# viniciusvidal2/slam-sensor-fusion

Hardware: AMD Instinct MI355X
Metric: scans_per_s_200k_scan_vs_10M_map (higher is better)
Workload: dtype f32 points / f64 accumulation

## Files before the change

### include/slamfusion.h

```cpp
#ifndef SLAMFUSION_H
#define SLAMFUSION_H
#include <stdint.h>

#ifdef __cplusplus
extern "C" {
#endif

#define SF_VERSION 210

typedef enum {
    SF_OK = 0,
    SF_ERR_INVALID = -1,
    SF_ERR_HIP = -2,
    SF_ERR_NOMEM = -3,
    SF_ERR_STATE = -4,
    SF_ERR_OVERFLOW = -5,
    SF_ERR_COMM = -6
} sf_status;

typedef struct sf_ctx sf_ctx;
typedef struct sf_cloud sf_cloud;
typedef struct sf_map sf_map;
typedef struct sf_icp sf_icp;

// ... 150 lines not shown
int sf_icp_align_batch_async(sf_icp *icp, int mode);
int sf_icp_fetch_results(sf_icp *icp, sf_icp_result *out);
int sf_icp_fetch_previous(sf_icp *icp, sf_icp_result *out);
int sf_icp_use_graph(sf_icp *icp, int on);
int sf_icp_graph_counts(sf_icp *icp, int64_t *captures, int64_t *launches);
int sf_icp_set_fused(sf_icp *icp, int on);
int sf_icp_fused_count(sf_icp *icp, int64_t *launches);
int sf_icp_fused_redone(sf_icp *icp, int64_t *redone);
int sf_icp_test_inject_barrier_timeout(sf_icp *icp);
#define SF_ORDER_AUTO 0
#define SF_ORDER_AS_GIVEN 1
#define SF_ORDER_CELL 2
int sf_icp_set_query_order(sf_icp *icp, int order);
int sf_icp_set_nn_reuse(sf_icp *icp, int on);
int sf_icp_set_wide_scan_points(sf_icp *icp, int64_t points);
int sf_icp_set_pipeline(sf_icp *icp, int on);
int sf_icp_set_tile_search(sf_icp *icp, int mode);
int sf_icp_tile_info(sf_icp *icp, int64_t out[12]);
int sf_icp_set_freeze(sf_icp *icp, int on);
int sf_icp_set_freeze_params(sf_icp *icp, float guard_scale, float guard_min, float guard_max, int max_tries, int from_launch);
int sf_icp_freeze_stats(sf_icp *icp, int64_t out[5]);
int sf_icp_set_defer_search(sf_icp *icp, int on);
int sf_icp_defer_stats(sf_icp *icp, int64_t out[2]);
int sf_icp_set_neighbour_research(sf_icp *icp, int from_launch);
int sf_icp_neighbour_stats(sf_icp *icp, int64_t out[3]);
int sf_icp_neighbour_gap_stats(sf_icp *icp, int64_t out[4]);
#define SF_ROBUST_NONE 0
#define SF_ROBUST_HUBER 1
#define SF_ROBUST_CAUCHY 2
#define SF_ROBUST_TUKEY 3
#define SF_ROBUST_GM 4
int sf_icp_set_robust_kernel(sf_icp *icp, int kind, double k);

#define SF_COV_EIG_EPS 1e-12
#define SF_COV_FEW_CORR 1
#define SF_COV_SINGULAR 2
#define SF_COV_DEGENERATE_TRANS 4
#define SF_COV_DEGENERATE_ROT 8
typedef struct {
    double info[36];
    double cov[36];
    double sigma2, sigma2_hat, weight_sum;
    double trans_info[3], trans_dir[9];
    double rot_info[3], rot_dir[9];
    int64_t n_corr;
    int32_t flags;
// ... 202 lines not shown
```

### slam_sensor_fusion_amd/api.py

```python
import atexit
import ctypes as C
import os
import weakref

import numpy as np

_HERE = os.path.dirname(os.path.abspath(__file__))
LIB_PATH = os.path.join(_HERE, "lib", "libslamfusion.so")

SF_ICP_REF_CPP, SF_ICP_O3D_P2P, SF_ICP_P2PLANE = 0, 1, 2
SF_VOXEL_PCL, SF_VOXEL_O3D, SF_VOXEL_PCL64 = 0, 1, 2
SF_FLAG_VOXEL_OVERFLOW = 1
SF_ICP_FLAG_FEW_CORR, SF_ICP_FLAG_SINGULAR, SF_ICP_FLAG_SHARD_STALE, SF_ICP_FLAG_BARRIER_TIMEOUT = 1, 2, 4, 8
PROF_NN, PROF_REDUCE, PROF_COLLECTIVE, PROF_SOLVE, PROF_SHARD_BUILD = 0, 1, 2, 3, 4
SF_ERR_COMM = -6
MODES = {"ref_cpp": SF_ICP_REF_CPP, "o3d_p2p": SF_ICP_O3D_P2P, "p2plane": SF_ICP_P2PLANE}
ROBUST_KINDS = {"none": 0, "huber": 1, "cauchy": 2, "tukey": 3, "gm": 4}


class SlamFusionError(RuntimeError):
    pass


class IcpResult(C.Structure):
# ... 782 lines not shown
        return {"froze": a[0], "thawed": a[1], "failed": a[2], "active_queries": a[3], "frozen_at_end": a[4]}

    def set_defer_search(self, on=True):
        _check(self.lib.sf_icp_set_defer_search(self.h, C.c_int(int(bool(on)))))

    def set_neighbour_research(self, from_launch=2):
        _check(self.lib.sf_icp_set_neighbour_research(self.h, C.c_int(int(from_launch))))

    def neighbour_stats(self):
        a = (C.c_int64 * 3)()
        _check(self.lib.sf_icp_neighbour_stats(self.h, a))
        return {"served": a[0], "not_served": a[1], "waves_searched": a[2]}

    def neighbour_gap_stats(self):
        a = (C.c_int64 * 4)()
        _check(self.lib.sf_icp_neighbour_gap_stats(self.h, a))
        return {"served": a[0], "not_served": a[1], "waves_searched": a[2], "by_gap": a[3]}

    def defer_stats(self):
        a = (C.c_int64 * 2)()
        _check(self.lib.sf_icp_defer_stats(self.h, a))
        return {"deferred_queries": a[0], "capped_waves": a[1]}

    def set_query_order(self, order="auto"):
        _check(self.lib.sf_icp_set_query_order(self.h, C.c_int({"auto": 0, "as_given": 1, "cell": 2}[order])))

    def align(self, mode="ref_cpp"):
        r = IcpResult()
        _check(self.lib.sf_icp_align(self.h, C.c_int(MODES[mode]), C.byref(r)))
        return r.as_dict()

    def align_batch(self, mode="p2plane"):
        arr = (IcpResult * self.batch)()
        _check(self.lib.sf_icp_align_batch(self.h, C.c_int(MODES[mode]), arr))
        self._prev_batch, self._last_batch = getattr(self, "_last_batch", None), self.batch
        return [r.as_dict() for r in arr]

    def align_batch_async(self, mode="p2plane"):
        _check(self.lib.sf_icp_align_batch_async(self.h, C.c_int(MODES[mode])))
        self._prev_batch, self._last_batch = getattr(self, "_last_batch", None), self.batch

    def fetch_results(self, raw=False):
        arr = (IcpResult * int(getattr(self, "_last_batch", None) or self.batch))()
        _check(self.lib.sf_icp_fetch_results(self.h, arr))
        return arr if raw else [r.as_dict() for r in arr]

# ... 639 lines not shown
```

### slam_sensor_fusion_amd/csrc/sf_icp.hip

```cpp
#include "sf_common.hpp"
#include "sf_nn.hpp"
#include "sf_tile.hpp"
#include "sf_order.hpp"
#include "sf_p2p.hpp"

#include <cfloat>
#include <cstdlib>
#include <cmath>
#include <vector>
#include <mutex>
#include <string>

namespace {

constexpr int BLK = 256;
constexpr int NREC_P2P = 17;
constexpr int NREC_PLANE = 30;
constexpr int REC_STRIDE = 32;

struct IcpState {
    double T[16];
    double rec[REC_STRIDE];
    double fitness, rmse, prev_fitness, prev_rmse;
    float last_error, err_pending;
// ... 1653 lines not shown
    const int r = (int)blockIdx.x, b = (int)blockIdx.y;
    if (A.st[b].done) return;
    const int fmode = A.fz[b].mode;
    if (fmode == 2) {
        const int64_t total = A.fz[b].n_active;
        for (int bx = r; (int64_t)bx * FZ_CAP < total; bx += FZ_FEW) {
            nn_red_fz_row<Q, SHARD>(g, w, A, b, bx, 2);
            __syncthreads();
        }
        return;
    }
    for (int bx = r; bx < A.nblocks; bx += FZ_FEW) {
        nn_red_fz_row<Q, SHARD>(g, w, A, b, bx, fmode);
        __syncthreads();
    }
}


#ifndef SF_DF_WCAP
#define SF_DF_WCAP 8
#endif
constexpr int DF_WCAP = SF_DF_WCAP;
constexpr int DF_CAPPED = 255;
static_assert((BLK / 64) * DF_WCAP <= FZ_CAP && DF_WCAP < DF_CAPPED, "a row defers fewer queries than it could list as active");
struct DeferBufs {
    uint8_t *cnt;
    uint16_t *ids;
    double *part;
    uint32_t *stat;
};

template <int Q>
__global__ __launch_bounds__(BLK, NN_RED_WAVES) void k_nn_red_df(SfGrid g, SfWindow w, const float *__restrict__ X0x, const float *__restrict__ X0y, const float *__restrict__ X0z,
                                                                 int n, const IcpState *__restrict__ st, float thr, double *__restrict__ partials, int nblocks,
                                                                 float4 *__restrict__ qcache, int64_t cache_n, uint32_t *__restrict__ stats, DeferBufs df)
{
    constexpr int MODE = 2;
    constexpr int NREC = NREC_PLANE;
    const int L = blockIdx.y * gridDim.x + blockIdx.x;
    const int kk = L >> 3;
    const int b = kk % (int)gridDim.y;
    const int bx = (L & 7) * ((int)gridDim.x >> 3) + kk / (int)gridDim.y;
    if (bx >= nblocks) return;
    const IcpState *S = st + b;
    if (S->done) return;
    __shared__ sf::WaveNN nn_ws[BLK / 64];
    __shared__ double stage[BLK / 64][32];
    const int wv = threadIdx.x >> 6, lane = threadIdx.x & 63;
    const size_t seg = ((size_t)b * nblocks + bx) * (BLK / 64) + wv;
    LanePair P[Q];
    bool need[Q];
#pragma unroll
    for (int u = 0; u < Q; ++u) need[u] = false;
    const bool attempted = qcache != nullptr && S->cache_live != 0 && S->n_research >= VERIFY_FROM_SEARCH;
    bool fast = false;
    uint32_t listed = 0;
    if (attempted) {
        const float m_now = (float)S->motion;
#pragma unroll
        for (int u = 0; u < Q; ++u) {
            const int slot = bx * (BLK * Q) + u * BLK + (int)threadIdx.x;
            const QueryIn q = query_in<MODE, false>(X0x, X0y, X0z, n, b, S, 0.0f, 0.0f, nullptr, qcache, cache_n, true, slot, n);
            sf::NNHit hit, seed;
            float4 tn;
            need[u] = reuse_certificate(q.valid, q.qx, q.qy, q.qz, thr, m_now, q.e, q.c1, q.c2, hit, tn, seed);
            if (g.nbr != nullptr && S->n_research >= g.nbr_from) {
                const bool tried = need[u] && seed.j >= 0;
                int served = 0;
                if (tried) {
                    served = table_serve<MODE>(g, q, thr, m_now, seed, qcache, cache_n, hit, tn);
                    need[u] = served == 0;
                }
                if (stats) table_count(stats, tried, served);
            }
            P[u] = make_pair(q, hit, tn);
        }
        uint32_t failing = 0;
// ... 98 lines not shown
                const LanePair A1 = nn_pair<MODE, false, false>(g, w, X0x, X0y, X0z, n, b, S, thr, 0.0f, 0.0f, nullptr, qcache, cache_n, slot, n, &nn_ws[wv], stats, nullptr, false);
#pragma unroll
                for (int h = 0; h < 2; ++h) {
                    double v[16];
#pragma unroll
                    for (int k = 0; k < 16; ++k) v[k] = 0.0;
                    const PairTerms t = pair_terms<MODE>(A1);
                    add_half<MODE>(t, h, v);
                    const double t0 = wave_reduce_16(v);
                    if ((lane & 3) == 0) fstage[wv][16 * h + (lane >> 2)] = t0;
                }
            } else if (lane < 32) {
                fstage[wv][lane] = 0.0;
            }
            __syncthreads();
            if (threadIdx.x < 32) acc += ((fstage[0][threadIdx.x] + fstage[1][threadIdx.x]) + fstage[2][threadIdx.x]) + fstage[3][threadIdx.x];
            __syncthreads();
        }
    }
    if (threadIdx.x < REC_STRIDE) df.part[((size_t)b * FZ_FEW + r) * REC_STRIDE + threadIdx.x] = threadIdx.x < NREC_PLANE ? acc : 0.0;
    __syncthreads();
    if (threadIdx.x == 0) {
        if (n_listed) atomicAdd(&df.stat[0], n_listed);
        if (capped) atomicAdd(&df.stat[1], capped);
    }
}

__device__ __forceinline__ void add_deferred_rows(const double *__restrict__ df_part, int b, double *rec)
{
    if (threadIdx.x < NREC_PLANE) {
        double v = 0.0;
#pragma unroll
        for (int r = 0; r < FZ_FEW; ++r) v += df_part[((size_t)b * FZ_FEW + r) * REC_STRIDE + threadIdx.x];
        rec[threadIdx.x] += v;
    }
    __syncthreads();
}

template <int STRIDE, int NCOL, int NT>
__device__ __forceinline__ void reduce_columns(const double *__restrict__ part, int nrows, double *out)
{
    constexpr int NS = 8;
    static_assert(NT % 128 == 0 && NT / 128 >= 1 && NT / 128 <= NS && NCOL <= 128, "slices of 128 columns");
    __shared__ double sl[NS][128];
    const int c = threadIdx.x & 127;
    for (int sidx = threadIdx.x >> 7; sidx < NS; sidx += NT / 128) {
        double v0 = 0, v1 = 0, v2 = 0, v3 = 0;
// ... 212 lines not shown
    const int b = blockIdx.x;
    IcpState *S = st + b;
    if (S->done) return;
    FreezeState *F = fb.fz + b;
    __shared__ double rec[REC_STRIDE];
    freeze_fold<RBLK>(S, F, b, partials, nblocks, nblocks, fb, rec);
    if (fb.df_part) add_deferred_rows(fb.df_part, b, rec);
    if (threadIdx.x == 0) {
        for (int c = 0; c < NREC_PLANE; ++c) S->rec[c] = rec[c];
        double To[12];
#pragma unroll
        for (int i = 0; i < 12; ++i) To[i] = S->T[i];
        const double m0 = S->motion;
        double upd[12];
        solve_plane(S, rec, n_src, K, upd);
        track_motion(S, To, boxp[b]);
        freeze_after_update(S, F, m0, S->motion, fp, request, upd);
    }
}

__global__ void k_fz_init(FreezeState *__restrict__ fz, int batch, uint32_t *__restrict__ df_stat)
{
    const int b = blockIdx.x * blockDim.x + threadIdx.x;
    if (b == 0) df_stat[0] = df_stat[1] = 0u;
    if (b >= batch) return;
    FreezeState *F = fz + b;
    F->mode = 0; F->tries = 0; F->froze = 0; F->thawed = 0; F->n_active = 0; F->guard = 0.0f; F->launch_mode = 0; F->motion0 = 0.0;
}

constexpr int SBLK = 256;
template <int MODE>
__global__ __launch_bounds__(SBLK) void k_reduce_only(IcpState *__restrict__ st, const double *__restrict__ partials, int nblocks, double *__restrict__ xchg,
                                                      const uint32_t *__restrict__ own_off, int qpl, FreezeBufs fb)
{
    constexpr int NREC = MODE == 2 ? NREC_PLANE : NREC_P2P;
    const int b = blockIdx.x;
    __shared__ double rec[REC_STRIDE];
    if (st[b].done) {
        if (threadIdx.x < REC_STRIDE) xchg[(size_t)b * REC_STRIDE + threadIdx.x] = 0.0;
        return;
    }
    const int rows = own_off ? (int)((own_off[b + 1] - own_off[b] + BLK * qpl - 1) / (BLK * qpl)) : nblocks;
    if (MODE == 2 && fb.fz) freeze_fold<SBLK>(st + b, fb.fz + b, b, partials, nblocks, rows, fb, rec);
    else reduce_partials<NREC, SBLK>(partials + (size_t)b * nblocks * REC_STRIDE, rows, rec);
    if (MODE == 2 && fb.df_part) add_deferred_rows(fb.df_part, b, rec);
    if (threadIdx.x < REC_STRIDE) xchg[(size_t)b * REC_STRIDE + threadIdx.x] = rec[threadIdx.x];
}
// ... 534 lines not shown
    int own_nblocks = 1;
    sf::DevBuf d_box;
    int last_mode = 0;
    bool fused = true;
    bool last_fused = false;
    sf::DevBuf bar;
    int fused_limit[4] = {-1, -1, -1, -1};
    double fused_share = 0.0;
    int64_t fused_redone = 0;
    bool inject_timeout = false;
    int64_t fused_launches = 0;
    IcpState *h_pin = nullptr;
    size_t h_pin_cap = 0;
    bool use_graph = false;
    int64_t graph_captures = 0, graph_replays = 0;
    struct GraphKey {
        int mode = -1, iters = -1, batch = -1, window = -1, ordered = -1, reuse = -1, robust_kind = -1, cov_on = -1;
        int64_t n = -1;
        const void *map = nullptr;
        uint64_t map_generation = 0, epochs = 0;
        uint64_t nbr_stamp = 0;
        const void *nbr = nullptr;
        int nbr_from = 0;
        float max_corr = 0, accept = 0, eps = 0;
        double robust_k = 0;
        double cov_prm[5] = {0, 0, 0, 0, 0};
        bool operator==(const GraphKey &o) const
        {
            return mode == o.mode && iters == o.iters && batch == o.batch && window == o.window && ordered == o.ordered && reuse == o.reuse && n == o.n && map == o.map &&
                   map_generation == o.map_generation && epochs == o.epochs && nbr_stamp == o.nbr_stamp && nbr == o.nbr && nbr_from == o.nbr_from && max_corr == o.max_corr && accept == o.accept && eps == o.eps &&
                   robust_kind == o.robust_kind && robust_k == o.robust_k && cov_on == o.cov_on && std::memcmp(cov_prm, o.cov_prm, sizeof(cov_prm)) == 0;
        }
    };
    struct LaneMeta {
        bool valid = false;
        bool cov = false;
        int batch = 0, mode = 0;
        std::vector<double> inits;
        int src_set = 0;
        uint64_t src_version = 0;
    };
    struct Lane {
        sf::DevBuf X;
        sf::DevBuf qcache;
        sf::DevBuf Xq, qkeys, qkeys2, qidx, qidx2;
        sf::DevBuf corr;
        sf::DevBuf state, d_inits, partials;
        sf::DevBuf fz_state, fz_part, fz_cnt, fz_ids, fz_all;
        sf::DevBuf df_cnt, df_ids, df_part, df_stat;
        sf::DevBuf qtkey, tseg, tile_stats;
        sf::DevBuf cov_part, cov_out;
        hipGraphExec_t graph_exec = nullptr;
        GraphKey graph_key;
// ... 48 lines not shown
    const void *mark_map = nullptr;
    SfWindow mark_window{};
    bool profiling = false;
    std::vector<hipEvent_t> ev;
    size_t ev_used = 0;
    int64_t prof_launches = 0;
    double prof_ms = 0;
    std::vector<float> prof_each;
    std::vector<int> ev_kind;
    std::vector<float> prof_phase[SF_PROF_KINDS];
    sf::DevBuf nn_stats;
    int freeze = 1;
    FreezeParams fz_prm{8.0f, 2.0e-5f, 3.0e-4f, 3};
    int fz_from = 5;
    bool fz_from_auto = true;
    int fz_fetches = 0;
    int fz_step = 0;
    int nbr_from = SF_NBR_FROM;
    bool nbr_active = false;
    int64_t nbr_stats_first = 0;
    uint64_t mark_nbr_stamp = 0;
    int defer = 1;
    bool df_planned = false;
    int64_t nn_stats_used = 0;
    static constexpr int64_t NN_STATS_CAP = 1024;
    int robust_kind = SF_ROBUST_NONE;
    double robust_k = 0.0;
    int cov_on = 0;
    CovArg cov_arg{0.0, 0.0, 0.0, 0.0, 0.0};
    bool prev_cov_ok = false;
    int tile_mode = 0;
    bool tile_on = false;
    sf::SfTiles tiles{};
};

namespace {

using Lane = sf_icp::Lane;
using SrcSet = sf_icp::SrcSet;
float *soa(sf::DevBuf &b, int64_t total, int axis) { return b.as<float>() + (size_t)axis * (size_t)total; }
const float *queries(sf_icp *icp, int axis)
{
    Lane &ln = icp->cur(); SrcSet &ss = icp->src();
    if (icp->shard) return soa(ln.Xq, icp->own_total, axis);
    return soa(icp->ordered ? ln.Xq : ss.X0, ss.plane, axis);
}
// ... 334 lines not shown
        (void)e;
    }
    ~ProfScope()
    {
        if (!icp->profiling) return;
        hipError_t e = hipEventRecord(icp->ev[icp->ev_used + 1], icp->ctx->stream);
        (void)e;
        icp->ev_used += 2;
    }
};

void prof_collect(sf_icp *icp)
{
    for (size_t k = 0; k + 1 < icp->ev_used; k += 2) {
        float ms = 0;
        if (hipEventElapsedTime(&ms, icp->ev[k], icp->ev[k + 1]) != hipSuccess) continue;
        const int kind = k / 2 < icp->ev_kind.size() ? icp->ev_kind[k / 2] : SF_PROF_NN;
        if (kind == SF_PROF_NN) { icp->prof_ms += ms; icp->prof_launches += 1; icp->prof_each.push_back(ms); }
        else if (kind > 0 && kind < SF_PROF_KINDS) icp->prof_phase[kind].push_back(ms);
    }
    icp->ev_used = 0;
}

sf_icp::GraphKey graph_key_now(const sf_icp *icp, int mode)
{
    const Lane &ln = icp->cur(); const SrcSet &ss = icp->src();
    sf_icp::GraphKey k;
    k.mode = mode; k.iters = icp->prm.num_iters; k.batch = ss.batch; k.window = icp->map->window.kind; k.ordered = (int)icp->ordered | ((int)icp->tile_on << 1); k.reuse = (int)icp->reuse | (icp->freeze << 1) | (icp->fz_from << 3) | (icp->defer << 16);
    k.n = (mode == SF_ICP_REF_CPP && ss.batch == 1) ? -ss.n_cap : ss.n;
    k.map = (const void *)icp->map;
    k.map_generation = icp->map->generation;
    if (icp->nbr_active) { k.nbr_stamp = icp->map->nbr_stamp; k.nbr = icp->map->nbr.p; k.nbr_from = icp->nbr_from; }
    k.robust_kind = robust_on(icp, mode) ? icp->robust_kind : SF_ROBUST_NONE; k.robust_k = robust_on(icp, mode) ? icp->robust_k : 0.0;
    k.cov_on = icp->cov_on;
    if (icp->cov_on) { const double cp[5] = {icp->cov_arg.sensor_sigma, icp->cov_arg.thr_t, icp->cov_arg.thr_r, icp->cov_arg.infl_t, icp->cov_arg.infl_r}; std::memcpy(k.cov_prm, cp, sizeof(cp)); }
    k.max_corr = icp->prm.max_corr; k.accept = icp->prm.accept; k.eps = icp->prm.eps + icp->fz_prm.guard_scale * 1.0e-3f + icp->fz_prm.guard_min + icp->fz_prm.guard_max + (float)icp->fz_prm.max_tries;
    const sf::DevBuf *bufs[] = {&ss.X0, &ss.X0r, &ln.X, &ln.Xq, &ln.qcache, &ln.corr, &ln.state, &ln.partials, &icp->d_box, &ss.d_boxes, &ss.n_dev,
                                &icp->map->pts4, &icp->map->nrm4, &icp->map->cell_start, &icp->map->d_window, &ln.fz_state, &ln.fz_part, &ln.fz_cnt, &ln.fz_ids, &ln.fz_all, &ln.df_cnt, &ln.df_ids, &ln.df_part, &ln.df_stat, &ln.tseg, &ln.tile_stats, &ln.cov_part, &ln.cov_out};
    k.epochs = (uint64_t)ss.plane;
    for (const sf::DevBuf *b : bufs) k.epochs = (k.epochs * 1000003ull + b->epoch) * 1000003ull + (uint64_t)(uintptr_t)b->p;
    return k;
}

SfGrid grid_for(const sf_icp *icp)
{
    SfGrid g = icp->map->grid;
    g.nbr = icp->nbr_active ? icp->map->nbr.as<uint4>() : nullptr;
    g.nbr_from = icp->nbr_from;
    return g;
}

int nbr_prepare(sf_icp *icp, int mode)
{
    sf_map *m = icp->map;
    const SrcSet &ss = icp->src();
// ... 83 lines not shown
}

bool freeze_on(const sf_icp *icp, int mode)
{
    const SrcSet &ss = icp->src();
    const int64_t nq = icp->shard ? icp->own_total : ss.n * ss.batch;
    const bool wanted = icp->freeze == 2 || (icp->freeze == 1 && nq >= FREEZE_AUTO_MIN_QUERIES);
    return mode == SF_ICP_P2PLANE && wanted && !robust_on(icp, mode) && icp->reuse && ss.qpl == SF_WIDE_QPL && icp->map->window.kind == 0 && icp->prm.num_iters > icp->fz_from + 1 &&
           icp->fz_from >= VERIFY_FROM_SEARCH;
}

int freeze_alloc(sf_icp *icp)
{
    Lane &ln = icp->cur(); SrcSet &ss = icp->src();
    const size_t rows = (size_t)ss.batch * (size_t)std::max(ss.nblocks_nn, icp->shard ? icp->own_nblocks : 0);
    SF_TRY(ln.fz_state.reserve(sizeof(FreezeState) * (size_t)ss.batch));
    SF_TRY(ln.fz_part.reserve(sizeof(double) * FZ_NMOM * rows));
    SF_TRY(ln.fz_cnt.reserve(sizeof(uint32_t) * rows));
    SF_TRY(ln.fz_ids.reserve(sizeof(uint16_t) * FZ_CAP * rows));
    SF_TRY(ln.fz_all.reserve(sizeof(uint32_t) * FZ_CAP * rows));
    SF_TRY(ln.df_cnt.reserve(sizeof(uint8_t) * (BLK / 64) * rows));
    SF_TRY(ln.df_ids.reserve(sizeof(uint16_t) * (BLK / 64) * DF_WCAP * rows));
    SF_TRY(ln.df_part.reserve(sizeof(double) * REC_STRIDE * FZ_FEW * (size_t)ss.batch));
    SF_TRY(ln.df_stat.reserve(sizeof(uint32_t) * 2));
    return SF_OK;
}

FreezeBufs freeze_bufs(sf_icp *icp, bool on, bool deferred = false)
{
    Lane &ln = icp->cur();
    FreezeBufs fb;
    fb.fz = on ? ln.fz_state.as<FreezeState>() : nullptr;
    fb.mom_part = ln.fz_part.as<double>();
    fb.act_cnt = ln.fz_cnt.as<uint32_t>();
    fb.act_ids = ln.fz_ids.as<uint16_t>();
    fb.act_all = ln.fz_all.as<uint32_t>();
    fb.df_part = deferred ? ln.df_part.as<double>() : nullptr;
    return fb;
}

DeferBufs defer_bufs(sf_icp *icp)
{
    Lane &ln = icp->cur();
    DeferBufs d;
    d.cnt = ln.df_cnt.as<uint8_t>();
    d.ids = ln.df_ids.as<uint16_t>();
    d.part = ln.df_part.as<double>();
    d.stat = ln.df_stat.as<uint32_t>();
    return d;
}

bool defer_now(const sf_icp *icp, int mode, int k)
{
    return freeze_on(icp, mode) && icp->defer != 0 && !icp->shard && k >= VERIFY_FROM_SEARCH && k + 1 == icp->fz_from;
}

bool defer_planned(const sf_icp *icp, int mode) { return defer_now(icp, mode, icp->fz_from - 1); }

void launch_nn_deferred(sf_icp *icp, uint32_t *stats)
{
    Lane &ln = icp->cur(); SrcSet &ss = icp->src();
    sf_map *m = icp->map;
    hipLaunchKernelGGL((k_nn_deferred<SF_WIDE_QPL>), dim3((unsigned)FZ_FEW, (unsigned)ss.batch), dim3(BLK), 0, icp->ctx->stream, grid_for(icp), m->window, queries(icp, 0), queries(icp, 1), queries(icp, 2),
                       (int)ss.n, ln.state.as<IcpState>(), o3d_thr(icp), ss.nblocks_nn, ln.qcache.as<float4>(), icp->cache_n, stats, defer_bufs(icp));
}

void launch_nn_red_df(sf_icp *icp)
{
    Lane &ln = icp->cur(); SrcSet &ss = icp->src();
    sf_map *m = icp->map;
    const int nb = ss.nblocks_nn;
    const dim3 grid((unsigned)((nb + 7) & ~7), (unsigned)ss.batch), blk(BLK);
    ProfScope ps(icp);
    uint32_t *stats = nullptr;
    if (icp->profiling && icp->nn_stats.p && icp->nn_stats_used < sf_icp::NN_STATS_CAP) stats = icp->nn_stats.as<uint32_t>() + NN_STATS_PER * NN_STATS_SHARDS * icp->nn_stats_used++;
    hipLaunchKernelGGL((k_nn_red_df<SF_WIDE_QPL>), grid, blk, 0, icp->ctx->stream, grid_for(icp), m->window, queries(icp, 0), queries(icp, 1), queries(icp, 2), (int)ss.n, ln.state.as<IcpState>(),
                       o3d_thr(icp), ln.partials.as<double>(), nb, ln.qcache.as<float4>(), icp->cache_n, stats, defer_bufs(icp));
    launch_nn_deferred(icp, stats);
}

void launch_nn_red_fz(sf_icp *icp, bool sharded, bool few)
{
    Lane &ln = icp->cur(); SrcSet &ss = icp->src();
    sf_map *m = icp->map;
    const int nb = sharded ? icp->own_nblocks : ss.nblocks_nn;
    const dim3 grid_full((unsigned)((nb + 7) & ~7), (unsigned)ss.batch), grid_few((unsigned)FZ_FEW, (unsigned)ss.batch), blk(BLK);
    ProfScope ps(icp);
    FzArgs A;
    A.X0x = queries(icp, 0); A.X0y = queries(icp, 1); A.X0z = queries(icp, 2);
    A.n = (int)ss.n;
    A.st = ln.state.as<IcpState>();
    A.thr = o3d_thr(icp); A.xlo = icp->xlo; A.xhi = icp->xhi;
    A.partials = ln.partials.as<double>();
    A.nblocks = nb;
    A.own_off = icp->own_off.as<uint32_t>();
    A.qcache = ln.qcache.as<float4>();
    A.cache_n = icp->cache_n;
    A.stats = nullptr;
    if (icp->profiling && icp->nn_stats.p && icp->nn_stats_used < sf_icp::NN_STATS_CAP) A.stats = icp->nn_stats.as<uint32_t>() + NN_STATS_PER * NN_STATS_SHARDS * icp->nn_stats_used++;
    A.fz = ln.fz_state.as<FreezeState>();
// ... 96 lines not shown
int enqueue_align(sf_icp *icp, int mode)
{
    Lane &ln = icp->cur(); SrcSet &ss = icp->src();
    sf_map *m = icp->map;
    hipStream_t s = icp->ctx->stream;
    IcpState *st = ln.state.as<IcpState>();
    double *part = ln.partials.as<double>();
    const int K = icp->prm.num_iters;
    const int B = ss.batch;
    const int n = (int)ss.n;
    if (mode == SF_ICP_O3D_P2P) {
        for (int k = 0; k <= K; ++k) {
            if (tile_launch(icp, k)) launch_tile_search<1>(icp, false);
            else launch_nn_red<1>(icp);
            hipLaunchKernelGGL(k_reduce_solve<1>, dim3(B), dim3(RBLK), 0, s, st, part, ss.nblocks_nn, n, k, K, ss.d_boxes.as<ScanBox>());
        }
    } else if (mode == SF_ICP_P2PLANE) {
        const bool fz = freeze_on(icp, mode);
        if (fz) {
            hipLaunchKernelGGL(k_fz_init, dim3(nblk(B, 64)), dim3(64), 0, s, ln.fz_state.as<FreezeState>(), B, ln.df_stat.as<uint32_t>());
        }
        const bool wide = ss.qpl > 1 && !icp->shard;
        for (int k = 0; k < K; ++k) {
            const bool q1 = wide && k < VERIFY_FROM_SEARCH;
            const bool df = !q1 && defer_now(icp, mode, k);
            if (fz && k >= icp->fz_from) launch_nn_red_fz(icp, false, k > icp->fz_from);
            else if (tile_launch(icp, k)) launch_tile_search<2>(icp, q1);
            else if (df) launch_nn_red_df(icp);
            else launch_nn_red<2>(icp, false, q1);
            if (fz && k + 1 >= icp->fz_from)
                hipLaunchKernelGGL(k_reduce_solve_fz, dim3(B), dim3(RBLK), 0, s, st, part, q1 ? ss.nblocks : ss.nblocks_nn, n, K, ss.d_boxes.as<ScanBox>(), freeze_bufs(icp, true, df),
                                   icp->fz_prm, (int)(k + 2 < K));
            else if (q1)
                hipLaunchKernelGGL(k_reduce_solve<2>, dim3(B), dim3(RBLK), 0, s, st, part, ss.nblocks, n, k, K, ss.d_boxes.as<ScanBox>());
            else
                hipLaunchKernelGGL(k_reduce_solve<2>, dim3(B), dim3(RBLK), 0, s, st, part, ss.nblocks_nn, n, k, K, ss.d_boxes.as<ScanBox>());
        }
    } else {
        SF_TRY(ln.X.reserve(sizeof(float) * 3 * (size_t)std::max<int64_t>(ss.plane, 1)));
        SF_TRY(ln.corr.reserve(sizeof(float4) * (size_t)std::max<int64_t>(ss.plane, 1)));
        float *Xx = soa(ln.X, ss.plane, 0), *Xy = soa(ln.X, ss.plane, 1), *Xz = soa(ln.X, ss.plane, 2);
        float4 *corr = ln.corr.as<float4>();
        const dim3 gpts((unsigned)ss.nblocks, (unsigned)B), gred((unsigned)ss.nblocks, (unsigned)B);
        const int *nl = B == 1 ? ss.n_dev.as<int>() : nullptr;
        const bool win = m->window.kind != 0;
        const float thr = icp->prm.max_corr;
        const dim3 gnn((unsigned)((ss.nblocks + 7) & ~7), (unsigned)B);
        auto nn = [&](int force) {
            ProfScope ps(icp);
            if (win) hipLaunchKernelGGL(k_ref_nn<true>, gnn, dim3(BLK), 0, s, m->grid, m->d_window.as<SfWindow>(), Xx, Xy, Xz, n, nl, st, thr, force, corr, ss.nblocks);
            else hipLaunchKernelGGL(k_ref_nn<false>, gnn, dim3(BLK), 0, s, m->grid, (const SfWindow *)nullptr, Xx, Xy, Xz, n, nl, st, thr, force, corr, ss.nblocks);
        };
        auto red = [&](int apply, int only_research) {
            hipLaunchKernelGGL(k_ref_red, gred, dim3(BLK), 0, s, Xx, Xy, Xz, n, nl, st, corr, apply, only_research, part, ss.nblocks);
        };
// ... 445 lines not shown
    for (int a = 0; a < 3; ++a) { out[1 + a] = icp->tiles.tc[a]; out[4 + a] = icp->tiles.nt[a]; }
    if (icp->cur().tile_stats.p) {
        SF_HIP(hipSetDevice(icp->ctx->device));
        unsigned long long h[TILE_STATS];
        SF_HIP(hipMemcpyAsync(h, icp->cur().tile_stats.p, sizeof(h), hipMemcpyDeviceToHost, icp->ctx->stream));
        SF_HIP(hipStreamSynchronize(icp->ctx->stream));
        for (int i = 0; i < 5; ++i) out[7 + i] = (int64_t)h[i];
    }
    return SF_OK;
}

extern "C" int sf_icp_set_defer_search(sf_icp *icp, int on)
{
    SF_CHECK(icp, SF_ERR_INVALID, "icp is NULL");
    icp->defer = on != 0;
    return SF_OK;
}

extern "C" int sf_icp_set_neighbour_research(sf_icp *icp, int from_launch)
{
    SF_CHECK(icp, SF_ERR_INVALID, "icp is NULL");
    SF_CHECK(from_launch != 0, SF_ERR_INVALID, "from_launch must be at least 1 (the first launch has no cached neighbours), or negative for off");
    icp->nbr_from = from_launch < 0 ? -1 : from_launch;
    return SF_OK;
}

namespace {
int neighbour_stats(sf_icp *icp, int64_t out[4])
{
    SF_CHECK(icp && out, SF_ERR_INVALID, "bad arguments");
    SF_CHECK(icp->profiling && icp->nn_stats.p, SF_ERR_STATE, "the neighbour statistics are counted in profiled runs (sf_icp_profile_enable)");
    SF_CHECK(icp->nn_stats_used < sf_icp::NN_STATS_CAP, SF_ERR_STATE, "the profiling counters are full (%lld launches since sf_icp_profile_enable): enable profiling again to reset them", (long long)sf_icp::NN_STATS_CAP);
    SF_HIP(hipStreamSynchronize(icp->ctx->stream));
    out[0] = out[1] = out[2] = out[3] = 0;
    const int64_t first = icp->nbr_stats_first, used = icp->nn_stats_used;
    if (used <= first) return SF_OK;
    const size_t per = (size_t)NN_STATS_PER * NN_STATS_SHARDS;
    std::vector<uint32_t> st(per * (size_t)(used - first), 0u);
    SF_HIP(hipMemcpy(st.data(), icp->nn_stats.as<uint32_t>() + per * (size_t)first, sizeof(uint32_t) * st.size(), hipMemcpyDeviceToHost));
    for (size_t i = 0; i < st.size(); i += NN_STATS_PER) { out[0] += st[i + 2]; out[1] += st[i + 3]; out[2] += st[i + 1]; out[3] += st[i + 4]; }
    return SF_OK;
}
}

extern "C" int sf_icp_neighbour_stats(sf_icp *icp, int64_t out[3])
{
    int64_t all[4];
    SF_CHECK(icp && out, SF_ERR_INVALID, "bad arguments");
    SF_TRY(neighbour_stats(icp, all));
    out[0] = all[0]; out[1] = all[1]; out[2] = all[2];
    return SF_OK;
}

extern "C" int sf_icp_neighbour_gap_stats(sf_icp *icp, int64_t out[4]) { return neighbour_stats(icp, out); }

extern "C" int sf_icp_defer_stats(sf_icp *icp, int64_t out[2])
{
    SF_CHECK(icp && out, SF_ERR_INVALID, "bad arguments");
    out[0] = out[1] = 0;
    if (!icp->df_planned || !icp->cur().df_stat.p) return SF_OK;
    uint32_t h[2] = {0u, 0u};
    SF_HIP(hipMemcpyAsync(h, icp->cur().df_stat.p, sizeof(h), hipMemcpyDeviceToHost, icp->ctx->stream));
    SF_HIP(hipStreamSynchronize(icp->ctx->stream));
    out[0] = (int64_t)h[0];
    out[1] = (int64_t)h[1];
    return SF_OK;
}

extern "C" int sf_icp_set_freeze(sf_icp *icp, int on)
{
    SF_CHECK(icp, SF_ERR_INVALID, "icp is NULL");
    SF_CHECK(on >= 0 && on <= 2, SF_ERR_INVALID, "sf_icp_set_freeze: 0 (off), 1 (auto) or 2 (always)");
    icp->freeze = on;
    return SF_OK;
}

namespace {
constexpr int FZ_FROM_DEFAULT = 5, FZ_PROBE_EVERY = 32;
void freeze_learn_schedule(sf_icp *icp)
{
    if (!icp->fz_from_auto || icp->last_fused || icp->shard || icp->last_mode != SF_ICP_P2PLANE) return;
    const int K = icp->prm.num_iters;
    if (++icp->fz_fetches >= FZ_PROBE_EVERY) { icp->fz_fetches = 0; icp->fz_from = FZ_FROM_DEFAULT; return; }
    if (!freeze_on(icp, icp->last_mode)) return;
    int latest = -1, never = 0;
    for (int b = 0; b < icp->src().batch; ++b) {
        const IcpState &S = icp->h_state[(size_t)b];
        if (S.froze_launch >= 0) latest = std::max(latest, S.froze_launch);
        else if (S.iterations >= K) never += 1;
    }
    if (latest < 0) icp->fz_from = std::max(FZ_FROM_DEFAULT, K);
    else if (never * 4 <= icp->src().batch) icp->fz_from = std::min(std::max(FZ_FROM_DEFAULT, latest), std::max(FZ_FROM_DEFAULT, K - 2));
}
}

extern "C" int sf_icp_set_robust_kernel(sf_icp *icp, int kind, double k)
{
    SF_CHECK(icp, SF_ERR_INVALID, "icp is NULL");
    SF_CHECK(kind >= SF_ROBUST_NONE && kind <= SF_ROBUST_GM, SF_ERR_INVALID, "unknown robust kernel %d", kind);
    SF_CHECK(kind == SF_ROBUST_NONE || (std::isfinite(k) && k > 0.0), SF_ERR_INVALID, "the robust kernel's scale must be finite and > 0 (got %g)", k);
    icp->robust_kind = kind;
    icp->robust_k = kind == SF_ROBUST_NONE ? 0.0 : k;
    return SF_OK;
}

extern "C" int sf_icp_set_freeze_params(sf_icp *icp, float guard_scale, float guard_min, float guard_max, int max_tries, int from_launch)
{
    SF_CHECK(icp, SF_ERR_INVALID, "icp is NULL");
    SF_CHECK(guard_scale >= 0.0f && guard_min >= 0.0f && guard_max >= guard_min && max_tries >= 0 && from_launch >= VERIFY_FROM_SEARCH && from_launch < 1024, SF_ERR_INVALID,
             "bad freeze parameters");
    icp->fz_prm = FreezeParams{guard_scale, guard_min, guard_max, max_tries};
    icp->fz_from = from_launch;
    icp->fz_from_auto = false;
    return SF_OK;
}

extern "C" int sf_icp_freeze_stats(sf_icp *icp, int64_t out[5])
{
    SF_CHECK(icp && out, SF_ERR_INVALID, "bad arguments");
    Lane &ln = icp->cur(); SrcSet &ss = icp->src();
    for (int i = 0; i < 5; ++i) out[i] = 0;
    if (!freeze_on(icp, icp->last_mode) || icp->last_fused || !ln.fz_state.p || ss.batch <= 0) return SF_OK;
    std::vector<FreezeState> h((size_t)ss.batch);
    SF_HIP(hipMemcpyAsync(h.data(), ln.fz_state.p, sizeof(FreezeState) * h.size(), hipMemcpyDeviceToHost, icp->ctx->stream));
    SF_HIP(hipStreamSynchronize(icp->ctx->stream));
    for (const FreezeState &f : h) {
        out[0] += f.froze;
        out[1] += f.thawed;
        out[2] += f.tries - f.thawed;
        out[3] += f.n_active;
        out[4] += f.mode == 2 ? 1 : 0;
    }
    return SF_OK;
}

extern "C" int sf_icp_graph_counts(sf_icp *icp, int64_t *captures, int64_t *launches)
// ... 129 lines not shown
}

int step_adopt_source(sf_icp *icp)
{
    SF_TRY(wait_src_ahead(icp, icp->ctx->stream));
    Lane &ln = icp->cur();
    const auto e0 = ln.state.epoch;
    SF_TRY(lane_reserve(icp));
    if (ln.state.epoch != e0) ln.meta.valid = false;
    SF_TRY(icp->xchg_own.reserve(sizeof(double) * REC_STRIDE * (size_t)std::max(icp->src().batch, 1)));
    icp->src_unmarked_use = true;
    return SF_OK;
}
}

extern "C" int sf_icp_align_batch_async(sf_icp *icp, int mode)
{
    SF_TRY(check_ready(icp, mode));
    SF_CHECK(!icp->shard, SF_ERR_STATE, "a sharded alignment needs the exchange between its halves: use sf_icp_step_begin / sf_icp_step_end");
    SF_HIP(hipSetDevice(icp->ctx->device));
    const SrcSet &ss = icp->src();
    icp->last_mode = mode;
    icp->last_fused = fused_eligible(icp, mode);
    icp->df_planned = !icp->last_fused && defer_planned(icp, mode);
    SF_TRY(order_lut_prepare(icp));
    SF_TRY(nbr_prepare(icp, mode));
    icp->nbr_stats_first = icp->nn_stats_used;
    const bool beside = icp->unfetched;
    LaneScope lanes(icp, icp->pipeline != 0 && !icp->last_fused && !icp->profiling && !ss.n_on_device);
    SF_TRY(lanes.rc);
    Lane &ln = icp->cur();
    if (!lanes.piped) SF_TRY(lane_reserve(icp));
    icp->unfetched = true;
    icp->prev_ok = lanes.piped && beside && icp->prev().meta.valid;
    icp->prev_cov_ok = icp->prev_ok && icp->prev().meta.cov;
    lane_describe(icp, mode, icp->cov_on != 0);
    hipStream_t s = icp->ctx->stream;
    if (icp->cov_on) SF_TRY(cov_alloc(icp));
    SF_TRY(launch_state_init(icp));
    if (icp->last_fused) {
        SF_TRY(order_queries(icp, mode));
        SF_TRY(launch_fused(icp, mode));
        if (icp->cov_on) {
            enqueue_cov(icp, mode, false);
            SF_HIP(hipGetLastError());
        }
        return SF_OK;
    }
    if (mode == SF_ICP_REF_CPP && icp->map->window.kind != 0) {
// ... 243 lines not shown
    if (own > 0) {
        hipLaunchKernelGGL(k_own_scatter, grid, dim3(BLK), 0, s, n, st, icp->own_keep.as<unsigned long long>(), icp->own_blk.as<uint32_t>(), nbf, icp->own_off.as<uint32_t>(),
                           icp->own_idx.as<uint32_t>());
        SF_TRY(run_order_sort(icp, B, (int64_t)maxc, own, icp->own_off.as<uint32_t>(), icp->own_idx.as<uint32_t>()));
    }
    hipLaunchKernelGGL(k_own_mark, dim3(nblk(B, 64)), dim3(64), 0, s, st, B);
    SF_HIP(hipGetLastError());
    return reuse_reset(icp, own);
}

}

extern "C" int sf_icp_step_begin(sf_icp *icp, int mode, int first)
{
    SF_TRY(check_ready(icp, mode));
    SF_CHECK(mode != SF_ICP_REF_CPP, SF_ERR_INVALID, "stepping supports O3D_P2P and P2PLANE");
    SF_CHECK(first >= 0 && first <= 2, SF_ERR_INVALID, "first must be 0, 1 or 2");
    SF_CHECK(!icp->cov_on, SF_ERR_STATE, COV_DECLINE_MSG);
    SF_CHECK(first != 2 || icp->shard, SF_ERR_STATE, "resume (first = 2) is a sharded-path operation");
    Lane &ln = icp->cur(); SrcSet &ss = icp->src();
    SF_HIP(hipSetDevice(icp->ctx->device));
    icp->last_mode = mode;
    icp->last_fused = false;
    icp->nbr_active = false;
    icp->map->served = true;
    if (first) SF_TRY(step_adopt_source(icp));
    if (first == 1) lane_describe(icp, mode, false);
    if (first) icp->df_planned = defer_planned(icp, mode);
    if (first) SF_TRY(order_lut_prepare(icp));
    if (first == 1) SF_TRY(launch_state_init(icp));
    if (icp->shard) {
        if (first) SF_TRY(shard_build(icp, first == 2));
    } else if (first) {
        SF_TRY(order_queries(icp, mode));
        SF_TRY(reuse_reset(icp, ss.n * ss.batch));
    }
    if (first) SF_TRY(freeze_start_pass(icp, mode));
    double *x = reinterpret_cast<double *>(sf_icp_exchange_ptr(icp, nullptr));
    hipStream_t s = icp->ctx->stream;
    const bool q1 = mode == SF_ICP_P2PLANE && ss.qpl > 1 && icp->fz_step < VERIFY_FROM_SEARCH;
    const int nb = icp->shard ? (q1 ? icp->own_nblocks * ss.qpl : icp->own_nblocks) : (q1 ? ss.nblocks : ss.nblocks_nn);
    const int qpl_now = q1 ? 1 : ss.qpl;
    const uint32_t *off = icp->shard ? icp->own_off.as<uint32_t>() : nullptr;
    if (mode == SF_ICP_O3D_P2P) {
        launch_nn_red<1>(icp, icp->shard);
        ProfScope ps(icp, SF_PROF_REDUCE);
        hipLaunchKernelGGL(k_reduce_only<1>, dim3(ss.batch), dim3(SBLK), 0, s, ln.state.as<IcpState>(), ln.partials.as<double>(), nb, x, off, ss.qpl, freeze_bufs(icp, false));
    } else {
        const bool df = !q1 && defer_now(icp, mode, icp->fz_step);
        if (freeze_nn_now(icp, mode)) launch_nn_red_fz(icp, icp->shard, icp->fz_step > icp->fz_from);
        else if (df) launch_nn_red_df(icp);
        else launch_nn_red<2>(icp, icp->shard, q1);
        ProfScope ps(icp, SF_PROF_REDUCE);
        hipLaunchKernelGGL(k_reduce_only<2>, dim3(ss.batch), dim3(SBLK), 0, s, ln.state.as<IcpState>(), ln.partials.as<double>(), nb, x, off, qpl_now,
                           freeze_bufs(icp, freeze_nn_now(icp, mode), df));
    }
    SF_HIP(hipGetLastError());
    return SF_OK;
}

extern "C" int sf_icp_step_end(sf_icp *icp, int mode, int last)
{
    SF_TRY(check_ready(icp, mode));
    Lane &ln = icp->cur(); SrcSet &ss = icp->src();
    (void)last;
    const double *x = reinterpret_cast<const double *>(sf_icp_exchange_ptr(icp, nullptr));
    hipStream_t s = icp->ctx->stream;
    const int K = icp->prm.num_iters;
    ProfScope ps(icp, SF_PROF_SOLVE);
    if (mode == SF_ICP_O3D_P2P)
        hipLaunchKernelGGL(k_solve_only<1>, dim3(nblk(ss.batch, 64)), dim3(64), 0, s, ln.state.as<IcpState>(), x, (int)ss.n, K, ss.batch, ss.d_boxes.as<ScanBox>(),
                           icp->shard ? icp->own_margin : 0.0f, (FreezeState *)nullptr, icp->fz_prm, 0);
// ... 280 lines not shown
```

Before: 21530.

## Extend deferred-search lookup to earlier launches when neighbour cache is active

Generalises the deferred nearest-neighbour path so it can start at the neighbour-research launch, before the last launch ahead of freeze, when neighbour caching is on. The aim is to skip full searches for more queries in earlier ICP iterations. Per-launch capped-wave counters are added, and the host reads them back to raise the first eligible launch when too many waves overflow the defer cap. This costs an extra device-to-host copy per fetch and a more complex launch schedule. It also threads neighbour state into the step API and adds a stats query.

```diff
diff --git a/include/slamfusion.h b/include/slamfusion.h
--- a/include/slamfusion.h
+++ b/include/slamfusion.h
@@ -196,6 +196,7 @@
 int sf_icp_freeze_stats(sf_icp *icp, int64_t out[5]);
 int sf_icp_set_defer_search(sf_icp *icp, int on);
 int sf_icp_defer_stats(sf_icp *icp, int64_t out[2]);
+int sf_icp_lookup_launch_stats(sf_icp *icp, int64_t out[4]);
 int sf_icp_set_neighbour_research(sf_icp *icp, int from_launch);
 int sf_icp_neighbour_stats(sf_icp *icp, int64_t out[3]);
 int sf_icp_neighbour_gap_stats(sf_icp *icp, int64_t out[4]);
diff --git a/slam_sensor_fusion_amd/api.py b/slam_sensor_fusion_amd/api.py
--- a/slam_sensor_fusion_amd/api.py
+++ b/slam_sensor_fusion_amd/api.py
@@ -828,6 +828,11 @@
         _check(self.lib.sf_icp_defer_stats(self.h, a))
         return {"deferred_queries": a[0], "capped_waves": a[1]}
 
+    def lookup_launch_stats(self):
+        a = (C.c_int64 * 4)()
+        _check(self.lib.sf_icp_lookup_launch_stats(self.h, a))
+        return {"launches": a[0], "deferred_queries": a[1], "capped_waves": a[2], "first": a[3]}
+
     def set_query_order(self, order="auto"):
         _check(self.lib.sf_icp_set_query_order(self.h, C.c_int({"auto": 0, "as_given": 1, "cell": 2}[order])))
 
diff --git a/slam_sensor_fusion_amd/csrc/sf_icp.hip b/slam_sensor_fusion_amd/csrc/sf_icp.hip
--- a/slam_sensor_fusion_amd/csrc/sf_icp.hip
+++ b/slam_sensor_fusion_amd/csrc/sf_icp.hip
@@ -1699,6 +1699,7 @@
 #endif
 constexpr int DF_WCAP = SF_DF_WCAP;
 constexpr int DF_CAPPED = 255;
+constexpr int DF_STAT_LAUNCHES = 32;
 static_assert((BLK / 64) * DF_WCAP <= FZ_CAP && DF_WCAP < DF_CAPPED, "a row defers fewer queries than it could list as active");
 struct DeferBufs {
     uint8_t *cnt;
@@ -1710,7 +1711,7 @@
 template <int Q>
 __global__ __launch_bounds__(BLK, NN_RED_WAVES) void k_nn_red_df(SfGrid g, SfWindow w, const float *__restrict__ X0x, const float *__restrict__ X0y, const float *__restrict__ X0z,
                                                                  int n, const IcpState *__restrict__ st, float thr, double *__restrict__ partials, int nblocks,
-                                                                 float4 *__restrict__ qcache, int64_t cache_n, uint32_t *__restrict__ stats, DeferBufs df)
+                                                                 float4 *__restrict__ qcache, int64_t cache_n, uint32_t *__restrict__ stats, DeferBufs df, int attempt_from)
 {
     constexpr int MODE = 2;
     constexpr int NREC = NREC_PLANE;
@@ -1729,7 +1730,7 @@
     bool need[Q];
 #pragma unroll
     for (int u = 0; u < Q; ++u) need[u] = false;
-    const bool attempted = qcache != nullptr && S->cache_live != 0 && S->n_research >= VERIFY_FROM_SEARCH;
+    const bool attempted = qcache != nullptr && S->cache_live != 0 && S->n_research >= attempt_from;
     bool fast = false;
     uint32_t listed = 0;
     if (attempted) {
@@ -1874,7 +1875,10 @@
     __syncthreads();
     if (threadIdx.x == 0) {
         if (n_listed) atomicAdd(&df.stat[0], n_listed);
-        if (capped) atomicAdd(&df.stat[1], capped);
+        if (capped) {
+            atomicAdd(&df.stat[1], capped);
+            atomicAdd(&df.stat[2 + min(max(S->n_research, 0), DF_STAT_LAUNCHES - 1)], capped);
+        }
     }
 }
 
@@ -2133,7 +2137,7 @@
 __global__ void k_fz_init(FreezeState *__restrict__ fz, int batch, uint32_t *__restrict__ df_stat)
 {
     const int b = blockIdx.x * blockDim.x + threadIdx.x;
-    if (b == 0) df_stat[0] = df_stat[1] = 0u;
+    if (b < 2 + DF_STAT_LAUNCHES) df_stat[b] = 0u;
     if (b >= batch) return;
     FreezeState *F = fz + b;
     F->mode = 0; F->tries = 0; F->froze = 0; F->thawed = 0; F->n_active = 0; F->guard = 0.0f; F->launch_mode = 0; F->motion0 = 0.0;
@@ -2714,13 +2718,14 @@
         uint64_t nbr_stamp = 0;
         const void *nbr = nullptr;
         int nbr_from = 0;
+        int defer_first = -1;
         float max_corr = 0, accept = 0, eps = 0;
         double robust_k = 0;
         double cov_prm[5] = {0, 0, 0, 0, 0};
         bool operator==(const GraphKey &o) const
         {
             return mode == o.mode && iters == o.iters && batch == o.batch && window == o.window && ordered == o.ordered && reuse == o.reuse && n == o.n && map == o.map &&
-                   map_generation == o.map_generation && epochs == o.epochs && nbr_stamp == o.nbr_stamp && nbr == o.nbr && nbr_from == o.nbr_from && max_corr == o.max_corr && accept == o.accept && eps == o.eps &&
+                   map_generation == o.map_generation && epochs == o.epochs && nbr_stamp == o.nbr_stamp && nbr == o.nbr && nbr_from == o.nbr_from && defer_first == o.defer_first && max_corr == o.max_corr && accept == o.accept && eps == o.eps &&
                    robust_kind == o.robust_kind && robust_k == o.robust_k && cov_on == o.cov_on && std::memcmp(cov_prm, o.cov_prm, sizeof(cov_prm)) == 0;
         }
     };
@@ -2815,6 +2820,10 @@
     uint64_t mark_nbr_stamp = 0;
     int defer = 1;
     bool df_planned = false;
+    int lk_first = -1, lk_launches = 0;
+    int64_t lk_waves = 0;
+    int lk_min = 0;
+    bool step_nbr = false;
     int64_t nn_stats_used = 0;
     static constexpr int64_t NN_STATS_CAP = 1024;
     int robust_kind = SF_ROBUST_NONE;
@@ -3195,6 +3204,8 @@
     icp->ev_used = 0;
 }
 
+int defer_first(const sf_icp *icp, int mode);
+
 sf_icp::GraphKey graph_key_now(const sf_icp *icp, int mode)
 {
     const Lane &ln = icp->cur(); const SrcSet &ss = icp->src();
@@ -3204,6 +3215,7 @@
     k.map = (const void *)icp->map;
     k.map_generation = icp->map->generation;
     if (icp->nbr_active) { k.nbr_stamp = icp->map->nbr_stamp; k.nbr = icp->map->nbr.p; k.nbr_from = icp->nbr_from; }
+    k.defer_first = defer_first(icp, mode);
     k.robust_kind = robust_on(icp, mode) ? icp->robust_kind : SF_ROBUST_NONE; k.robust_k = robust_on(icp, mode) ? icp->robust_k : 0.0;
     k.cov_on = icp->cov_on;
     if (icp->cov_on) { const double cp[5] = {icp->cov_arg.sensor_sigma, icp->cov_arg.thr_t, icp->cov_arg.thr_r, icp->cov_arg.infl_t, icp->cov_arg.infl_r}; std::memcpy(k.cov_prm, cp, sizeof(cp)); }
@@ -3333,7 +3345,7 @@
     SF_TRY(ln.df_cnt.reserve(sizeof(uint8_t) * (BLK / 64) * rows));
     SF_TRY(ln.df_ids.reserve(sizeof(uint16_t) * (BLK / 64) * DF_WCAP * rows));
     SF_TRY(ln.df_part.reserve(sizeof(double) * REC_STRIDE * FZ_FEW * (size_t)ss.batch));
-    SF_TRY(ln.df_stat.reserve(sizeof(uint32_t) * 2));
+    SF_TRY(ln.df_stat.reserve(sizeof(uint32_t) * (2 + DF_STAT_LAUNCHES)));
     return SF_OK;
 }
 
@@ -3361,12 +3373,34 @@
     return d;
 }
 
-bool defer_now(const sf_icp *icp, int mode, int k)
-{
-    return freeze_on(icp, mode) && icp->defer != 0 && !icp->shard && k >= VERIFY_FROM_SEARCH && k + 1 == icp->fz_from;
-}
-
-bool defer_planned(const sf_icp *icp, int mode) { return defer_now(icp, mode, icp->fz_from - 1); }
+int lookup_first(const sf_icp *icp, int mode)
+{
+    if (!freeze_on(icp, mode) || icp->defer == 0 || icp->shard || !icp->nbr_active || icp->nbr_from < 1) return icp->fz_from;
+    return std::min(icp->fz_from, std::max(icp->nbr_from, icp->lk_min));
+}
+
+bool lookup_form(const sf_icp *icp, int mode) { return lookup_first(icp, mode) < icp->fz_from; }
+
+int defer_first(const sf_icp *icp, int mode)
+{
+    if (!freeze_on(icp, mode) || icp->defer == 0 || icp->shard) return icp->fz_from;
+    const int last = icp->fz_from - 1 >= VERIFY_FROM_SEARCH ? icp->fz_from - 1 : icp->fz_from;
+    return std::min(lookup_first(icp, mode), last);
+}
+
+bool defer_now(const sf_icp *icp, int mode, int k) { return k >= defer_first(icp, mode) && k < icp->fz_from; }
+
+bool defer_planned(const sf_icp *icp, int mode) { return defer_first(icp, mode) < icp->fz_from; }
+
+bool one_per_lane_now(const sf_icp *icp, int mode, int k) { return mode == SF_ICP_P2PLANE && icp->src().qpl > 1 && k < VERIFY_FROM_SEARCH && !defer_now(icp, mode, k); }
+
+void lookup_describe(sf_icp *icp, int mode)
+{
+    const bool on = !icp->last_fused && lookup_form(icp, mode);
+    icp->lk_first = on ? lookup_first(icp, mode) : -1;
+    icp->lk_launches = on ? icp->fz_from - icp->lk_first : 0;
+    icp->lk_waves = (int64_t)icp->src().batch * icp->src().nblocks_nn * (BLK / 64);
+}
 
 void launch_nn_deferred(sf_icp *icp, uint32_t *stats)
 {
@@ -3386,7 +3420,8 @@
     uint32_t *stats = nullptr;
     if (icp->profiling && icp->nn_stats.p && icp->nn_stats_used < sf_icp::NN_STATS_CAP) stats = icp->nn_stats.as<uint32_t>() + NN_STATS_PER * NN_STATS_SHARDS * icp->nn_stats_used++;
     hipLaunchKernelGGL((k_nn_red_df<SF_WIDE_QPL>), grid, blk, 0, icp->ctx->stream, grid_for(icp), m->window, queries(icp, 0), queries(icp, 1), queries(icp, 2), (int)ss.n, ln.state.as<IcpState>(),
-                       o3d_thr(icp), ln.partials.as<double>(), nb, ln.qcache.as<float4>(), icp->cache_n, stats, defer_bufs(icp));
+                       o3d_thr(icp), ln.partials.as<double>(), nb, ln.qcache.as<float4>(), icp->cache_n, stats, defer_bufs(icp),
+                       lookup_form(icp, SF_ICP_P2PLANE) ? lookup_first(icp, SF_ICP_P2PLANE) : VERIFY_FROM_SEARCH);
     launch_nn_deferred(icp, stats);
 }
 
@@ -3529,15 +3564,15 @@
         }
         const bool wide = ss.qpl > 1 && !icp->shard;
         for (int k = 0; k < K; ++k) {
-            const bool q1 = wide && k < VERIFY_FROM_SEARCH;
-            const bool df = !q1 && defer_now(icp, mode, k);
+            const bool df = defer_now(icp, mode, k);
+            const bool q1 = wide && k < VERIFY_FROM_SEARCH && !df;
             if (fz && k >= icp->fz_from) launch_nn_red_fz(icp, false, k > icp->fz_from);
+            else if (df) launch_nn_red_df(icp);
             else if (tile_launch(icp, k)) launch_tile_search<2>(icp, q1);
-            else if (df) launch_nn_red_df(icp);
             else launch_nn_red<2>(icp, false, q1);
-            if (fz && k + 1 >= icp->fz_from)
+            if (fz && (df || k + 1 >= icp->fz_from))
                 hipLaunchKernelGGL(k_reduce_solve_fz, dim3(B), dim3(RBLK), 0, s, st, part, q1 ? ss.nblocks : ss.nblocks_nn, n, K, ss.d_boxes.as<ScanBox>(), freeze_bufs(icp, true, df),
-                                   icp->fz_prm, (int)(k + 2 < K));
+                                   icp->fz_prm, (int)(k + 1 >= icp->fz_from && k + 2 < K));
             else if (q1)
                 hipLaunchKernelGGL(k_reduce_solve<2>, dim3(B), dim3(RBLK), 0, s, st, part, ss.nblocks, n, k, K, ss.d_boxes.as<ScanBox>());
             else
@@ -4029,6 +4064,7 @@
     SF_CHECK(icp, SF_ERR_INVALID, "icp is NULL");
     SF_CHECK(from_launch != 0, SF_ERR_INVALID, "from_launch must be at least 1 (the first launch has no cached neighbours), or negative for off");
     icp->nbr_from = from_launch < 0 ? -1 : from_launch;
+    icp->lk_min = 0;
     return SF_OK;
 }
 
@@ -4074,6 +4110,21 @@
     return SF_OK;
 }
 
+extern "C" int sf_icp_lookup_launch_stats(sf_icp *icp, int64_t out[4])
+{
+    SF_CHECK(icp && out, SF_ERR_INVALID, "bad arguments");
+    out[0] = out[1] = out[2] = 0;
+    out[3] = -1;
+    if (icp->lk_launches <= 0) return SF_OK;
+    int64_t df[2];
+    SF_TRY(sf_icp_defer_stats(icp, df));
+    out[0] = icp->lk_launches;
+    out[1] = df[0];
+    out[2] = df[1];
+    out[3] = icp->lk_first;
+    return SF_OK;
+}
+
 extern "C" int sf_icp_set_freeze(sf_icp *icp, int on)
 {
     SF_CHECK(icp, SF_ERR_INVALID, "icp is NULL");
@@ -4088,8 +4139,15 @@
 {
     if (!icp->fz_from_auto || icp->last_fused || icp->shard || icp->last_mode != SF_ICP_P2PLANE) return;
     const int K = icp->prm.num_iters;
-    if (++icp->fz_fetches >= FZ_PROBE_EVERY) { icp->fz_fetches = 0; icp->fz_from = FZ_FROM_DEFAULT; return; }
+    if (++icp->fz_fetches >= FZ_PROBE_EVERY) { icp->fz_fetches = 0; icp->fz_from = FZ_FROM_DEFAULT; icp->lk_min = 0; return; }
     if (!freeze_on(icp, icp->last_mode)) return;
+    if (icp->lk_launches > 0 && icp->cur().df_stat.p) {
+        uint32_t h[2 + DF_STAT_LAUNCHES];
+        if (hipMemcpy(h, icp->cur().df_stat.p, sizeof(h), hipMemcpyDeviceToHost) == hipSuccess) {
+            for (int k = icp->lk_first; k < icp->lk_first + icp->lk_launches && k < DF_STAT_LAUNCHES - 1; ++k)
+                if ((int64_t)h[2 + k] * 8 > icp->lk_waves) icp->lk_min = std::max(icp->lk_min, k + 1);
+        }
+    }
     int latest = -1, never = 0;
     for (int b = 0; b < icp->src().batch; ++b) {
         const IcpState &S = icp->h_state[(size_t)b];
@@ -4119,6 +4177,7 @@
     icp->fz_prm = FreezeParams{guard_scale, guard_min, guard_max, max_tries};
     icp->fz_from = from_launch;
     icp->fz_from_auto = false;
+    icp->lk_min = 0;
     return SF_OK;
 }
 
@@ -4294,9 +4353,10 @@
     const SrcSet &ss = icp->src();
     icp->last_mode = mode;
     icp->last_fused = fused_eligible(icp, mode);
-    icp->df_planned = !icp->last_fused && defer_planned(icp, mode);
     SF_TRY(order_lut_prepare(icp));
     SF_TRY(nbr_prepare(icp, mode));
+    icp->df_planned = !icp->last_fused && defer_planned(icp, mode);
+    lookup_describe(icp, mode);
     icp->nbr_stats_first = icp->nn_stats_used;
     const bool beside = icp->unfetched;
     LaneScope lanes(icp, icp->pipeline != 0 && !icp->last_fused && !icp->profiling && !ss.n_on_device);
@@ -4586,11 +4646,16 @@
     SF_HIP(hipSetDevice(icp->ctx->device));
     icp->last_mode = mode;
     icp->last_fused = false;
-    icp->nbr_active = false;
+    if (first) {
+        SF_TRY(nbr_prepare(icp, mode));
+        icp->step_nbr = icp->nbr_active;
+        icp->nbr_stats_first = icp->nn_stats_used;
+    }
+    icp->nbr_active = icp->step_nbr;
     icp->map->served = true;
     if (first) SF_TRY(step_adopt_source(icp));
     if (first == 1) lane_describe(icp, mode, false);
-    if (first) icp->df_planned = defer_planned(icp, mode);
+    if (first) { icp->df_planned = defer_planned(icp, mode); lookup_describe(icp, mode); }
     if (first) SF_TRY(order_lut_prepare(icp));
     if (first == 1) SF_TRY(launch_state_init(icp));
     if (icp->shard) {
@@ -4602,7 +4667,7 @@
     if (first) SF_TRY(freeze_start_pass(icp, mode));
     double *x = reinterpret_cast<double *>(sf_icp_exchange_ptr(icp, nullptr));
     hipStream_t s = icp->ctx->stream;
-    const bool q1 = mode == SF_ICP_P2PLANE && ss.qpl > 1 && icp->fz_step < VERIFY_FROM_SEARCH;
+    const bool q1 = one_per_lane_now(icp, mode, icp->fz_step);
     const int nb = icp->shard ? (q1 ? icp->own_nblocks * ss.qpl : icp->own_nblocks) : (q1 ? ss.nblocks : ss.nblocks_nn);
     const int qpl_now = q1 ? 1 : ss.qpl;
     const uint32_t *off = icp->shard ? icp->own_off.as<uint32_t>() : nullptr;
@@ -4611,7 +4676,7 @@
         ProfScope ps(icp, SF_PROF_REDUCE);
         hipLaunchKernelGGL(k_reduce_only<1>, dim3(ss.batch), dim3(SBLK), 0, s, ln.state.as<IcpState>(), ln.partials.as<double>(), nb, x, off, ss.qpl, freeze_bufs(icp, false));
     } else {
-        const bool df = !q1 && defer_now(icp, mode, icp->fz_step);
+        const bool df = mode == SF_ICP_P2PLANE && defer_now(icp, mode, icp->fz_step);
         if (freeze_nn_now(icp, mode)) launch_nn_red_fz(icp, icp->shard, icp->fz_step > icp->fz_from);
         else if (df) launch_nn_red_df(icp);
         else launch_nn_red<2>(icp, icp->shard, q1);
```

Result: faster. 22060, median of 6 (+2.5%).
